# apache/arrow-go

Hardware: AMD Instinct MI355X
Metric: GB/s processed per kernel (Sum/Add/Filter/Take) vs HBM roofline (higher is better)
Workload: dtype int64+f64

## Files before the change

### arrow_go_amd/csrc/ah_common.h

```cpp
#pragma once
#include <hip/hip_runtime.h>
#include <initializer_list>
#include <type_traits>
#include <stdarg.h>
#include <stdint.h>
#include <stddef.h>
#include <stdio.h>
#include <stdlib.h>
#include <string.h>
#include "../../include/arrowhip.h"

#define AH_EXPORT extern "C" __attribute__((visibility("default")))

struct ah_filter_cache {
  bool valid;
  const uint8_t *fdata, *fvalid;
  int64_t foff, n, ntiles;
  int null_sel, tile_rows;
  void* buf;
  size_t bytes;
  int64_t* super_off;
  int* tile_local;
  int64_t* total;
};
// ... 4 lines not shown
  hipStream_t copy_stream;
  bool owns_stream;
  hipEvent_t ev_copy;
  hipEvent_t ev_compute;
  hipEvent_t t0, t1;
  hipEvent_t* marks;
  int n_marks;
  void* scratch;
  size_t scratch_bytes;
  void* temp;
  size_t temp_bytes;
  uint64_t* pinned;
  uint64_t* dscalars;
  int num_cu;
  int tune_nt;
  int tune_blocks_per_cu;
  int opt_take_binned, opt_take_window_log2, opt_take_gather_wg, opt_take_gather_load, opt_take_gather_lds;
  int opt_groupby_keys;
  int opt_groupby_partition;
  int opt_encode_partition;
  int opt_encode_part_slots;
  int opt_encode_byte_map;
  int opt_encode_early_look;
  int opt_encode_part_min;
  int opt_hash_direct;
  int opt_sort_msd;
  int opt_scan_segment_log2;
  void* expr_cache;
  int capturing;
  ah_filter_cache fcache;
  int opt_scan_onepass;
  void* scan_recs;
  size_t scan_recs_bytes;
  unsigned scan_epoch;
  int opt_groupby_seed;
  int opt_groupby_reserve;
  int opt_groupby_lean;
  int opt_filter_cache;
  int take_clustered_hint;
  int opt_take_vec;
  bool take_hint_valid, take_hint_live;
  const void* take_hint_idx; int64_t take_hint_nidx; int take_hint_kind, take_hint_near, take_hint_uses, opt_take_hint_cache;
  unsigned long long take_hint_word;
  int opt_arith_xcd_map;
  int opt_groupby_scale_guess;
  int opt_encode_unperm2_group;
  int opt_encode_resolve_wgs;
  int opt_encode_dict_compact;
  int opt_encode_table_batch;
  int opt_encode_unperm_group;
  int opt_take_vec_nt;
  unsigned long long* mailbox;
  unsigned long long mailbox_seq;
  char err[512];
};

static inline unsigned ah_stream_grid(const ah_ctx* c, int64_t work_items, int default_bpc = 8) {
  int bpc = c->tune_blocks_per_cu > 0 ? c->tune_blocks_per_cu : default_bpc;
  int64_t cap = bpc > 0 ? (int64_t)c->num_cu * bpc : ((int64_t)1 << 30);
  int64_t g = work_items < cap ? work_items : cap;
  return (unsigned)(g < 1 ? 1 : g);
}

static inline int ah_fail(ah_ctx* ctx, int code, const char* fmt, ...) __attribute__((format(printf, 3, 4)));
static inline int ah_fail(ah_ctx* ctx, int code, const char* fmt, ...) {
  if (ctx) {
    va_list ap;
    va_start(ap, fmt);
    vsnprintf(ctx->err, sizeof(ctx->err), fmt, ap);
    va_end(ap);
  }
  return code;
}

#define AH_HIP(ctx, call)                                                              \
  do {                                                                                 \
    hipError_t e__ = (call);                                                           \
    if (e__ != hipSuccess)                                                             \
      return ah_fail((ctx), AH_EHIP, "%s failed: %s (%s:%d)", #call, hipGetErrorString(e__), \
                     __FILE__, __LINE__);                                              \
  } while (0)

#define AH_ENTER_KEEP(ctx)                                             \
  do {                                                                 \
    if (!(ctx)) return AH_EINVALID;                                    \
    (ctx)->err[0] = 0;                                                 \
    AH_HIP((ctx), hipSetDevice((ctx)->device));                        \
  } while (0)

#define AH_ENTER(ctx)                                                  \
  do {                                                                 \
    AH_ENTER_KEEP(ctx);                                                \
    (ctx)->fcache.valid = false;                                       \
    (ctx)->take_hint_valid = false;                                    \
  } while (0)

static inline bool ah_take_hint_overlaps(const ah_ctx* c, const void* p, size_t nbytes) {
  if (!c->take_hint_valid || !c->take_hint_idx) return false;
  const uintptr_t a = (uintptr_t)p, b = a + nbytes, lo = (uintptr_t)c->take_hint_idx, hi = lo + (size_t)c->take_hint_nidx * (size_t)(c->take_hint_kind / 2);
  return a < hi && lo < b;
}
static inline bool ah_fcache_overlaps(const ah_ctx* c, const void* p, size_t nbytes) {
  if (!c->fcache.valid) return false;
  const uintptr_t a = (uintptr_t)p, b = a + nbytes;
  const uintptr_t lo = (uintptr_t)(c->fcache.foff >> 3), hi = (uintptr_t)((c->fcache.foff + c->fcache.n + 7) >> 3);
  for (const uint8_t* bm : {c->fcache.fdata, c->fcache.fvalid})
// ... 131 lines not shown
  for (int j = 0; j < (int)(16 / sizeof(T)); j++) raw[j] = x.v[j];
  __builtin_nontemporal_store(raw, reinterpret_cast<ah_raw16<T>*>(p));
}

template <typename T>
__device__ __forceinline__ ah_vec16<T> ah_ld16(const T* p) {
  const ah_raw16<T> raw = *reinterpret_cast<const ah_raw16<T>*>(p);
  ah_vec16<T> r;
#pragma unroll
  for (int j = 0; j < (int)(16 / sizeof(T)); j++) r.v[j] = raw[j];
  return r;
}
template <typename T>
__device__ __forceinline__ void ah_st16(T* p, const ah_vec16<T>& x) {
  ah_raw16<T> raw;
#pragma unroll
  for (int j = 0; j < (int)(16 / sizeof(T)); j++) raw[j] = x.v[j];
  *reinterpret_cast<ah_raw16<T>*>(p) = raw;
}

template <typename T>
using ah_aligned16 = T __attribute__((ext_vector_type(16 / sizeof(T))));
template <typename ST>
__device__ __forceinline__ ah_vec16<ST> ah_load16(const ST* base, int64_t i, bool aligned) {
  ah_vec16<ST> v;
  if (aligned) {
    const ah_aligned16<ST> t = __builtin_nontemporal_load((const ah_aligned16<ST>*)base + i);
    __builtin_memcpy(&v, &t, 16);
  } else {
    v = ah_ld16<ST>(base + i * (int64_t)(16 / sizeof(ST)));
  }
  return v;
}
template <typename ST>
__device__ __forceinline__ void ah_store16(ST* base, int64_t i, const ah_vec16<ST>& v, bool aligned) {
  if (aligned) {
    ah_aligned16<ST> t;
    __builtin_memcpy(&t, &v, 16);
    __builtin_nontemporal_store(t, (ah_aligned16<ST>*)base + i);
  } else {
    ah_st16<ST>(base + i * (int64_t)(16 / sizeof(ST)), v);
  }
}

template <typename T>
__device__ __forceinline__ T ah_wave_sum(T v) {
#pragma unroll
  for (int o = 32; o > 0; o >>= 1) v += __shfl_down(v, o, 64);
  return v;
}

__device__ __forceinline__ int ah_lane() { return (int)(threadIdx.x & 63); }

__device__ __forceinline__ int ah_bit(const uint8_t* __restrict__ bm, int64_t i) {
  return bm == nullptr ? 1 : (bm[i >> 3] >> (i & 7)) & 1;
}

__device__ __forceinline__ uint64_t ah_load_bits64(const uint8_t* __restrict__ bm, int64_t pos, int nvalid);
__device__ __forceinline__ uint64_t ah_wave_bits64(const uint8_t* __restrict__ bm, int64_t pos0, int64_t nrows_left) {
  const int64_t p = ((int64_t)__builtin_amdgcn_readfirstlane((int)(pos0 >> 32)) << 32) | (unsigned)__builtin_amdgcn_readfirstlane((int)pos0);
  const int64_t left = ((int64_t)__builtin_amdgcn_readfirstlane((int)(nrows_left >> 32)) << 32) | (unsigned)__builtin_amdgcn_readfirstlane((int)nrows_left);
  return ah_load_bits64(bm, p, left >= 64 ? 64 : (int)(left < 0 ? 0 : left));
}
__device__ __forceinline__ uint64_t ah_load_bits64(const uint8_t* __restrict__ bm, int64_t pos, int nvalid) {
  uint64_t mask = nvalid >= 64 ? ~0ull : ((1ull << nvalid) - 1);
  if (nvalid <= 0) return 0;
  if (bm == nullptr) return mask;
  uintptr_t addr = (uintptr_t)bm + (uintptr_t)(pos >> 3);
  uintptr_t base = addr & ~(uintptr_t)7;
  int shift = (int)((addr - base) * 8 + (pos & 7));
  const uint64_t* w = (const uint64_t*)base;
  uint64_t lo = w[0] >> shift;
  if (shift != 0 && shift + nvalid > 64) lo |= w[1] << (64 - shift);
  return lo & mask;
}

__device__ __forceinline__ void put_bits(uint8_t* __restrict__ bm, int64_t pos, unsigned long long word, int cnt) {
  const uintptr_t addr = (uintptr_t)bm + (uintptr_t)(pos >> 3);
  const int sub = (int)(pos & 7);
  if (cnt == 64 && sub == 0 && (addr & 7) == 0) {
    *(unsigned long long*)addr = word;
    return;
  }
  const uintptr_t base = addr & ~(uintptr_t)3;
  int shift = (int)((addr - base) * 8) + sub;
  const unsigned long long m = cnt >= 64 ? ~0ull : ((1ull << cnt) - 1);
  word &= m;
  unsigned* w = (unsigned*)base;
  const unsigned long long mlo = m << shift, vlo = word << shift;
  const unsigned long long mhi = shift ? (m >> (64 - shift)) : 0ull, vhi = shift ? (word >> (64 - shift)) : 0ull;
  const unsigned m0 = (unsigned)mlo, m1 = (unsigned)(mlo >> 32), m2 = (unsigned)mhi;
  const unsigned v0 = (unsigned)vlo, v1 = (unsigned)(vlo >> 32), v2 = (unsigned)vhi;
  if (m0) { atomicAnd(&w[0], ~m0); if (v0) atomicOr(&w[0], v0); }
  if (m1) { atomicAnd(&w[1], ~m1); if (v1) atomicOr(&w[1], v1); }
  if (m2) { atomicAnd(&w[2], ~m2); if (v2) atomicOr(&w[2], v2); }
}

__device__ __forceinline__ void put_word(uint8_t* __restrict__ out, int64_t out_off, int aligned, int64_t chunk, unsigned long long word, int cnt) {
  if (aligned && cnt == 64) *(unsigned long long*)(out + (out_off + chunk * 64) / 8) = word;
  else put_bits(out, out_off + chunk * 64, word, cnt);
}

__device__ __forceinline__ void put_chunk_bytes(uint8_t* __restrict__ bm, int64_t chunk, int64_t n, unsigned long long word) {
  const int64_t left = n - chunk * 64;
  const int nbytes = left >= 64 ? 8 : (int)((left + 7) >> 3);
  for (int b = 0; b < nbytes; b++) bm[chunk * 8 + b] = (uint8_t)(word >> (8 * b));
// ... 2 lines not shown
```

### arrow_go_amd/csrc/ah_ctx.hip

```cpp
#include <chrono>
#include "ah_common.h"

static const char* kVersion = "arrowhip 0.1 (gfx950)";

AH_EXPORT const char* ah_version(void) { return kVersion; }

AH_EXPORT int ah_device_count(int* n_host) {
  int n = 0;
  hipError_t e = hipGetDeviceCount(&n);
  if (n_host) *n_host = (e == hipSuccess) ? n : 0;
  return e == hipSuccess ? AH_OK : AH_EHIP;
}

static int ctx_init_common(ah_ctx* c) {
  AH_HIP(c, hipStreamCreateWithFlags(&c->copy_stream, hipStreamNonBlocking));
  AH_HIP(c, hipEventCreateWithFlags(&c->ev_copy, hipEventDisableTiming));
  AH_HIP(c, hipEventCreateWithFlags(&c->ev_compute, hipEventDisableTiming));
  AH_HIP(c, hipEventCreate(&c->t0));
  AH_HIP(c, hipEventCreate(&c->t1));
  AH_HIP(c, hipHostMalloc((void**)&c->pinned, 64 * sizeof(uint64_t), hipHostMallocDefault));
  AH_HIP(c, hipMalloc((void**)&c->dscalars, (64 + 4096) * sizeof(uint64_t)));
  AH_HIP(c, hipMemset(c->dscalars, 0, (64 + 4096) * sizeof(uint64_t)));
  AH_HIP(c, hipHostMalloc((void**)&c->mailbox, 256, hipHostMallocCoherent | hipHostMallocMapped));
  memset(c->mailbox, 0, 256);
  hipDeviceProp_t prop;
  AH_HIP(c, hipGetDeviceProperties(&prop, c->device));
  c->num_cu = prop.multiProcessorCount > 0 ? prop.multiProcessorCount : 256;
  const char* e_nt = getenv("ARROWHIP_NT");
  c->tune_nt = e_nt ? atoi(e_nt) : 1;
  const char* e_bpc = getenv("ARROWHIP_BLOCKS_PER_CU");
  c->tune_blocks_per_cu = e_bpc ? atoi(e_bpc) : 0;
  auto env_int = [](const char* name, int dflt) { const char* e = getenv(name); return e ? atoi(e) : dflt; };
  c->opt_take_binned = env_int("ARROWHIP_TAKE_BINNED", 1);
  c->opt_take_window_log2 = env_int("ARROWHIP_TAKE_WINDOW_LOG2", 22);
  c->opt_take_gather_wg = env_int("ARROWHIP_TAKE_GATHER_WG_PER_CU", 8);
  c->opt_groupby_partition = env_int("ARROWHIP_GROUPBY_PARTITION", 1);
  c->opt_groupby_keys = env_int("ARROWHIP_GROUPBY_KEYS", 1280);
  c->opt_hash_direct = env_int("ARROWHIP_HASH_DIRECT", 2);
  c->opt_encode_partition = env_int("ARROWHIP_ENCODE_PARTITION", 1);
  c->opt_encode_part_min = env_int("ARROWHIP_ENCODE_PART_MIN", 300000);
  c->opt_encode_early_look = env_int("ARROWHIP_ENCODE_EARLY_LOOK", 1);
  c->opt_encode_byte_map = env_int("ARROWHIP_ENCODE_BYTE_MAP", 1);
  c->opt_encode_part_slots = env_int("ARROWHIP_ENCODE_PART_SLOTS", 8192);
  c->opt_sort_msd = env_int("ARROWHIP_SORT_MSD", 1);
  c->opt_scan_segment_log2 = env_int("ARROWHIP_SCAN_SEGMENT_LOG2", 0);
  c->opt_take_gather_lds = env_int("ARROWHIP_TAKE_GATHER_LDS", 1);
  c->opt_take_vec_nt = env_int("ARROWHIP_TAKE_VEC_NT", 7);
  c->opt_encode_unperm_group = env_int("ARROWHIP_ENCODE_UNPERM_GROUP", 4);
  c->opt_encode_table_batch = env_int("ARROWHIP_ENCODE_TABLE_BATCH", 1);
  c->opt_encode_dict_compact = env_int("ARROWHIP_ENCODE_DICT_COMPACT", 1);
  c->opt_encode_resolve_wgs = env_int("ARROWHIP_ENCODE_RESOLVE_WGS", 1024);
  c->opt_encode_unperm2_group = env_int("ARROWHIP_ENCODE_UNPERM2_GROUP", 4);
  c->opt_groupby_scale_guess = env_int("ARROWHIP_GROUPBY_SCALE_GUESS", 1);
  c->opt_arith_xcd_map = env_int("ARROWHIP_ARITH_XCD_MAP", 0);
  c->opt_take_vec = env_int("ARROWHIP_TAKE_VEC", 1);
  c->opt_take_gather_load = env_int("ARROWHIP_TAKE_GATHER_LOAD", 0);
  return AH_OK;
}

static int ctx_create(int device_id, void* stream, bool borrow, ah_ctx** out) {
  if (!out) return AH_EINVALID;
  *out = nullptr;
  ah_ctx* c = (ah_ctx*)calloc(1, sizeof(ah_ctx));
  if (!c) return AH_EINVALID;
  c->device = device_id;
  hipError_t e = hipSetDevice(device_id);
  if (e != hipSuccess) { free(c); return AH_EHIP; }
  if (borrow) {
    c->stream = (hipStream_t)stream;
    c->owns_stream = false;
  } else {
    e = hipStreamCreateWithFlags(&c->stream, hipStreamNonBlocking);
    if (e != hipSuccess) { free(c); return AH_EHIP; }
    c->owns_stream = true;
  }
  int rc = ctx_init_common(c);
  if (rc != AH_OK) { fprintf(stderr, "arrowhip: ctx init failed: %s\n", c->err); free(c); return rc; }
  c->opt_filter_cache = c->owns_stream ? 1 : 0;
  c->opt_take_hint_cache = c->owns_stream ? 1 : 0;
  c->opt_groupby_lean = 1;
  c->opt_scan_onepass = 1;
  c->opt_groupby_seed = 1;
  c->opt_groupby_reserve = 1;
  *out = c;
  return AH_OK;
}

AH_EXPORT int ah_ctx_create(int device_id, ah_ctx** out) { return ctx_create(device_id, nullptr, false, out); }
AH_EXPORT int ah_ctx_create_on_stream(int device_id, void* hip_stream, ah_ctx** out) {
  return ctx_create(device_id, hip_stream, true, out);
}

AH_EXPORT void ah_ctx_destroy(ah_ctx* c) {
  if (!c) return;
  (void)hipSetDevice(c->device);
  (void)hipStreamSynchronize(c->stream);
  (void)hipStreamSynchronize(c->copy_stream);
  ah_expr_cache_free(c);
  if (c->scratch) (void)hipFree(c->scratch);
  if (c->pinned) (void)hipHostFree(c->pinned);
  if (c->dscalars) (void)hipFree(c->dscalars);
  if (c->mailbox) (void)hipHostFree(c->mailbox);
  if (c->fcache.buf) (void)hipFree(c->fcache.buf);
  if (c->scan_recs) (void)hipFree(c->scan_recs);
  if (c->temp) (void)hipFree(c->temp);
  (void)hipEventDestroy(c->ev_copy);
  (void)hipEventDestroy(c->ev_compute);
  (void)hipEventDestroy(c->t0);
  (void)hipEventDestroy(c->t1);
  for (int i = 0; i < c->n_marks; i++) if (c->marks[i]) (void)hipEventDestroy(c->marks[i]);
  free(c->marks);
  (void)hipStreamDestroy(c->copy_stream);
  if (c->owns_stream) (void)hipStreamDestroy(c->stream);
  free(c);
}

AH_EXPORT int ah_ctx_set_option(ah_ctx* c, const char* name, int64_t value) {
  AH_ENTER(c);
  if (!name) return ah_fail(c, AH_EINVALID, "set_option: null name");
  if (!strcmp(name, "nt")) c->tune_nt = (int)value;
  else if (!strcmp(name, "blocks_per_cu")) c->tune_blocks_per_cu = (int)value;
  else if (!strcmp(name, "take_binned")) c->opt_take_binned = (int)value;
  else if (!strcmp(name, "take_window_log2")) c->opt_take_window_log2 = (int)value;
  else if (!strcmp(name, "take_gather_wg_per_cu")) c->opt_take_gather_wg = (int)value;
  else if (!strcmp(name, "take_gather_lds")) c->opt_take_gather_lds = (int)value;
  else if (!strcmp(name, "take_vec")) c->opt_take_vec = (int)value;
  else if (!strcmp(name, "take_hint_cache")) { c->opt_take_hint_cache = (int)value; c->take_hint_valid = false; }
  else if (!strcmp(name, "take_vec_nt")) c->opt_take_vec_nt = (int)value;
  else if (!strcmp(name, "encode_unperm_group")) c->opt_encode_unperm_group = (int)value;
  else if (!strcmp(name, "encode_table_batch")) c->opt_encode_table_batch = (int)value;
  else if (!strcmp(name, "encode_dict_compact")) c->opt_encode_dict_compact = (int)value;
  else if (!strcmp(name, "encode_unperm2_group")) c->opt_encode_unperm2_group = (int)value;
  else if (!strcmp(name, "encode_resolve_wgs")) c->opt_encode_resolve_wgs = value < 1 ? 1 : (int)value;
  else if (!strcmp(name, "groupby_scale_guess")) c->opt_groupby_scale_guess = (int)value;
  else if (!strcmp(name, "arith_xcd_map")) c->opt_arith_xcd_map = (int)value;
  else if (!strcmp(name, "take_gather_load")) c->opt_take_gather_load = (int)value;
  else if (!strcmp(name, "groupby_partition")) c->opt_groupby_partition = (int)value;
  else if (!strcmp(name, "groupby_keys")) c->opt_groupby_keys = (int)value;
  else if (!strcmp(name, "hash_direct")) c->opt_hash_direct = (int)value;
  else if (!strcmp(name, "encode_partition")) c->opt_encode_partition = (int)value;
  else if (!strcmp(name, "encode_part_min")) c->opt_encode_part_min = (int)value;
  else if (!strcmp(name, "encode_early_look")) c->opt_encode_early_look = (int)value;
  else if (!strcmp(name, "encode_byte_map")) c->opt_encode_byte_map = (int)value;
  else if (!strcmp(name, "encode_part_slots")) c->opt_encode_part_slots = (int)value;
  else if (!strcmp(name, "sort_msd")) c->opt_sort_msd = (int)value;
  else if (!strcmp(name, "scan_onepass")) c->opt_scan_onepass = (int)value;
  else if (!strcmp(name, "groupby_lean")) c->opt_groupby_lean = (int)value;
  else if (!strcmp(name, "groupby_seed")) c->opt_groupby_seed = (int)value;
  else if (!strcmp(name, "groupby_reserve")) c->opt_groupby_reserve = (int)value;
  else if (!strcmp(name, "filter_cache")) { c->opt_filter_cache = value != 0; if (!value) c->fcache.valid = false; }
  else if (!strcmp(name, "scan_segment_log2")) c->opt_scan_segment_log2 = (int)value;
  else return ah_fail(c, AH_EINVALID, "set_option: unknown option '%s'", name);
  return AH_OK;
}

AH_EXPORT const char* ah_last_error(ah_ctx* c) { return c ? c->err : "null context"; }

namespace {
__global__ void mailbox_post_kernel(const unsigned long long* __restrict__ src, int nwords, const unsigned long long* __restrict__ src2, int nwords2,
                                    unsigned long long* mailbox, unsigned long long seq) {
  for (int i = 0; i < nwords; i++) __hip_atomic_store(&mailbox[i], src[i], __ATOMIC_RELAXED, __HIP_MEMORY_SCOPE_SYSTEM);
  for (int i = 0; i < nwords2; i++) __hip_atomic_store(&mailbox[nwords + i], src2[i], __ATOMIC_RELAXED, __HIP_MEMORY_SCOPE_SYSTEM);
  __hip_atomic_store(&mailbox[7], seq, __ATOMIC_RELEASE, __HIP_MEMORY_SCOPE_SYSTEM);
}
}
int ah_mailbox_read(ah_ctx* c, const unsigned long long* dev_words, int nwords, unsigned long long* out_host) {
  return ah_mailbox_read2(c, dev_words, nwords, nullptr, 0, out_host);
}
int ah_mailbox_begin(ah_ctx* c, unsigned long long** mb_out, unsigned long long* seq_out) {
  if (c->capturing) { c->capturing = 2; return ah_fail(c, AH_EINVALID, "this call returns a value to the host: it cannot be recorded into a graph"); }
  *mb_out = c->mailbox + 8;
  *seq_out = ++c->mailbox_seq;
  return AH_OK;
}
int ah_mailbox_wait(ah_ctx* c, unsigned long long seq, int nwords, unsigned long long* out_host) {
  if (nwords < 1 || nwords > 7) return ah_fail(c, AH_EINVALID, "mailbox_wait: 1..7 words");
  unsigned long long* mb = c->mailbox + 8;
  bool seen = false;
  const auto t0 = std::chrono::steady_clock::now();
  for (unsigned spin = 0;; spin++) {
    if (__atomic_load_n(&mb[7], __ATOMIC_ACQUIRE) == seq) { seen = true; break; }
    __builtin_ia32_pause();
    if ((spin & 1023u) == 1023u && std::chrono::steady_clock::now() - t0 > std::chrono::milliseconds(5)) break;
  }
  if (!seen) {
    AH_HIP(c, hipStreamSynchronize(c->stream));
    if (__atomic_load_n(&mb[7], __ATOMIC_ACQUIRE) != seq) return ah_fail(c, AH_EHIP, "mailbox_wait: the kernel did not report");
  }
  for (int i = 0; i < nwords; i++) out_host[i] = __atomic_load_n(&mb[i], __ATOMIC_RELAXED);
  return AH_OK;
}
int ah_mailbox_read2(ah_ctx* c, const unsigned long long* dev_words, int nwords, const unsigned long long* dev_words2, int nwords2,
                     unsigned long long* out_host) {
  if (nwords < 1 || nwords2 < 0 || nwords + nwords2 > 7) return ah_fail(c, AH_EINVALID, "mailbox_read: 1..7 words");
  if (c->capturing) { c->capturing = 2; return ah_fail(c, AH_EINVALID, "this call returns a value to the host: it cannot be recorded into a graph"); }
  unsigned long long* mb = c->mailbox + 8;
  const unsigned long long seq = ++c->mailbox_seq;
  mailbox_post_kernel<<<1, 1, 0, c->stream>>>(dev_words, nwords, dev_words2, nwords2, mb, seq);
// ... 303 lines not shown
```

### arrow_go_amd/csrc/ah_fused.hip

```cpp
#include "ah_common.h"
#include "ah_ddsum.h"

namespace {

constexpr int kBlock = 256;
constexpr int kUnroll = 4;

template <typename T>
using Vec2 = T __attribute__((ext_vector_type(2)));

template <typename T, int OP>
__device__ __forceinline__ bool pred(T a, T t) {
  if (OP == AH_CMP_EQ) return a == t;
  if (OP == AH_CMP_NE) return a != t;
  if (OP == AH_CMP_GT) return a > t;
  return a >= t;
}

struct PartF64 { ah_ddx a; unsigned long long n; };
struct PartI64 { unsigned long long s; unsigned long long n; };

template <typename T> struct Acc;
template <> struct Acc<double> {
  using Part = PartF64;
// ... 30 lines not shown
  }
  __device__ __forceinline__ Part part() const { return Part{s, n}; }
};

template <typename T>
__device__ __forceinline__ void block_reduce(Acc<T>& a, typename Acc<T>::Part* out) {
  __shared__ typename Acc<T>::Part sm[kBlock / 64];
  a.wave_reduce();
  if ((threadIdx.x & 63) == 0) sm[threadIdx.x >> 6] = a.part();
  __syncthreads();
  if (threadIdx.x == 0) {
    Acc<T> r;
#pragma unroll
    for (int w = 0; w < kBlock / 64; w++) r.merge(sm[w]);
    *out = r.part();
  }
}

template <typename T, int OP, bool HAS_VALID, bool NT, bool CAREFUL>
__device__ __forceinline__ unsigned fused_walk(const Vec2<T>* __restrict__ body, int64_t row0, int64_t nvec,
                                               const uint8_t* __restrict__ valid, int64_t off, T thr, Acc<T>& a) {
  unsigned top = 0;
  const int64_t n_iters = (nvec + (int64_t)kBlock * kUnroll - 1) / ((int64_t)kBlock * kUnroll);
  for (int64_t it = blockIdx.x; it < n_iters; it += gridDim.x) {
    const int64_t base = it * kBlock * kUnroll + threadIdx.x;
    const bool full = (it + 1) * (int64_t)kBlock * kUnroll <= nvec;
    Vec2<T> v[kUnroll];
    if (full) {
#pragma unroll
      for (int k = 0; k < kUnroll; k++) {
        if (NT) v[k] = __builtin_nontemporal_load(&body[base + (int64_t)k * kBlock]);
        else v[k] = body[base + (int64_t)k * kBlock];
      }
    }
#pragma unroll
    for (int k = 0; k < kUnroll; k++) {
      const int64_t j = base + (int64_t)k * kBlock;
      if (!full) {
        if (j >= nvec) continue;
        v[k] = body[j];
      }
      unsigned vb = 3;
      if (HAS_VALID) {
        const int64_t bit = off + row0 + 2 * j;
        vb = (unsigned)((valid[bit >> 3] >> (bit & 7)) & 1) | ((unsigned)((valid[(bit + 1) >> 3] >> ((bit + 1) & 7)) & 1) << 1);
      }
      if ((vb & 1) && pred<T, OP>(v[k].x, thr)) { if (CAREFUL) a.add(v[k].x); else top = max(top, a.add_small(v[k].x)); }
      if ((vb & 2) && pred<T, OP>(v[k].y, thr)) { if (CAREFUL) a.add(v[k].y); else top = max(top, a.add_small(v[k].y)); }
    }
  }
  return top;
}

template <typename T, int OP, bool HAS_VALID, bool NT>
__global__ __launch_bounds__(kBlock) void fused_kernel(const T* __restrict__ x, int64_t n, int64_t row0, int64_t nvec,
                                                        const uint8_t* __restrict__ valid, int64_t off, T thr,
                                                        typename Acc<T>::Part* __restrict__ partials) {
  Acc<T> a;
  const Vec2<T>* body = (const Vec2<T>*)(x + row0);
  const unsigned top = fused_walk<T, OP, HAS_VALID, NT, !Acc<T>::kClassed>(body, row0, nvec, valid, off, thr, a);
  if (Acc<T>::kClassed && __any(top >= AH_DDX_BIG_HI)) {
    a = Acc<T>();
    (void)fused_walk<T, OP, HAS_VALID, NT, true>(body, row0, nvec, valid, off, thr, a);
  }
  if (blockIdx.x == 0 && threadIdx.x == 0) {
    for (int64_t i = 0; i < row0; i++)
      if ((!HAS_VALID || ah_bit(valid, off + i)) && pred<T, OP>(x[i], thr)) a.add(x[i]);
    for (int64_t i = row0 + 2 * nvec; i < n; i++)
      if ((!HAS_VALID || ah_bit(valid, off + i)) && pred<T, OP>(x[i], thr)) a.add(x[i]);
  }
  block_reduce<T>(a, &partials[blockIdx.x]);
}

template <typename T>
__global__ __launch_bounds__(kBlock) void fused_final_kernel(const typename Acc<T>::Part* __restrict__ partials, int np,
                                                              T* __restrict__ out_sum, int64_t* __restrict__ out_count,
                                                              double* __restrict__ out_parts) {
  Acc<T> a;
  for (int i = threadIdx.x; i < np; i += kBlock) a.merge(partials[i]);
  __shared__ typename Acc<T>::Part res;
  block_reduce<T>(a, &res);
  __syncthreads();
  if (threadIdx.x == 0) {
    if constexpr (__is_floating_point(T)) {
      *out_sum = ah_ddx_result(res.a);
      if (out_parts) { out_parts[0] = res.a.s; out_parts[1] = res.a.e; out_parts[2] = res.a.bs; out_parts[3] = res.a.be; }
    } else {
      *out_sum = (T)res.s;
    }
    *out_count = (int64_t)res.n;
  }
}

template <typename T>
int fused_dev(ah_ctx* c, int cmpop, const T* x, const uint8_t* valid, int64_t off, int64_t n, T thr, T* out_sum_dev,
              int64_t* out_count_dev, double* out_parts_dev = nullptr) {
  if (n < 0 || off < 0) return ah_fail(c, AH_EINVALID, "cmp_filter_sum: negative length/offset");
  if (n == 0) {
    AH_HIP(c, hipMemsetAsync(out_sum_dev, 0, sizeof(T), c->stream));
    AH_HIP(c, hipMemsetAsync(out_count_dev, 0, sizeof(int64_t), c->stream));
    if (out_parts_dev) AH_HIP(c, hipMemsetAsync(out_parts_dev, 0, 4 * sizeof(double), c->stream));
    return AH_OK;
  }
  if (!x) return ah_fail(c, AH_EINVALID, "cmp_filter_sum: null values");
  if ((uintptr_t)x & 7) return ah_fail(c, AH_EINVALID, "cmp_filter_sum: buffer not element-aligned");
  int64_t row0 = ((uintptr_t)x & 15) ? 1 : 0;
  if (row0 > n) row0 = n;
  int64_t nvec = (n - row0) / 2;
  unsigned grid = ah_stream_grid(c, ah_ceil_div(nvec > 0 ? nvec : 1, (int64_t)kBlock * kUnroll), valid ? 8 : 2);
  using Part = typename Acc<T>::Part;
  void* scratch;
  int rc = ah_scratch_reserve(c, (size_t)grid * sizeof(Part), &scratch);
  if (rc != AH_OK) return rc;
  Part* partials = (Part*)scratch;
#define AH_FUSED(OPC)                                                                                                   \
  if (valid) {                                                                                                          \
    if (c->tune_nt) fused_kernel<T, OPC, true, true><<<grid, kBlock, 0, c->stream>>>(x, n, row0, nvec, valid, off, thr, partials);   \
    else fused_kernel<T, OPC, true, false><<<grid, kBlock, 0, c->stream>>>(x, n, row0, nvec, valid, off, thr, partials);             \
  } else {                                                                                                              \
    if (c->tune_nt) fused_kernel<T, OPC, false, true><<<grid, kBlock, 0, c->stream>>>(x, n, row0, nvec, valid, off, thr, partials);  \
    else fused_kernel<T, OPC, false, false><<<grid, kBlock, 0, c->stream>>>(x, n, row0, nvec, valid, off, thr, partials);            \
  }
  switch (cmpop) {
    case AH_CMP_EQ: AH_FUSED(AH_CMP_EQ) break;
    case AH_CMP_NE: AH_FUSED(AH_CMP_NE) break;
    case AH_CMP_GT: AH_FUSED(AH_CMP_GT) break;
    case AH_CMP_GE: AH_FUSED(AH_CMP_GE) break;
    default: return ah_fail(c, AH_EINVALID, "cmp_filter_sum: bad op %d", cmpop);
  }
#undef AH_FUSED
  AH_LAUNCH_CHECK(c);
  fused_final_kernel<T><<<1, kBlock, 0, c->stream>>>(partials, (int)grid, out_sum_dev, out_count_dev, out_parts_dev);
  AH_LAUNCH_CHECK(c);
  return AH_OK;
}

template <typename T>
int fused_host(ah_ctx* c, int cmpop, const T* x, const uint8_t* valid, int64_t off, int64_t n, T thr, T* out_sum_host,
               int64_t* out_count_host) {
  T* dsum = (T*)&c->dscalars[8];
  int64_t* dcnt = (int64_t*)&c->dscalars[9];
  int rc = fused_dev<T>(c, cmpop, x, valid, off, n, thr, dsum, dcnt);
  if (rc != AH_OK) return rc;
  { int mrc = ah_mailbox_read(c, (const unsigned long long*)dsum, 2, (unsigned long long*)c->pinned); if (mrc != AH_OK) return mrc; }
  if (out_sum_host) memcpy(out_sum_host, (const void*)&c->pinned[0], sizeof(T));
  if (out_count_host) memcpy(out_count_host, (const void*)&c->pinned[1], sizeof(int64_t));
  return AH_OK;
}

}

AH_EXPORT int ah_cmp_filter_sum_i64(ah_ctx* c, int cmpop, const int64_t* x, const uint8_t* valid, int64_t off, int64_t n,
                                    int64_t threshold, int64_t* out_sum_host, int64_t* out_count_host) {
  AH_ENTER(c);
  return fused_host<int64_t>(c, cmpop, x, valid, off, n, threshold, out_sum_host, out_count_host);
}
AH_EXPORT int ah_cmp_filter_sum_f64(ah_ctx* c, int cmpop, const double* x, const uint8_t* valid, int64_t off, int64_t n,
                                    double threshold, double* out_sum_host, int64_t* out_count_host) {
  AH_ENTER(c);
  return fused_host<double>(c, cmpop, x, valid, off, n, threshold, out_sum_host, out_count_host);
}
AH_EXPORT int ah_cmp_filter_sum_i64_dev(ah_ctx* c, int cmpop, const int64_t* x, const uint8_t* valid, int64_t off,
                                        int64_t n, int64_t threshold, int64_t* out_sum_count_dev) {
  AH_ENTER(c);
  if (!out_sum_count_dev) return ah_fail(c, AH_EINVALID, "cmp_filter_sum: null output");
  return fused_dev<int64_t>(c, cmpop, x, valid, off, n, threshold, out_sum_count_dev, out_sum_count_dev + 1);
}
AH_EXPORT int ah_cmp_filter_sum_f64_dev(ah_ctx* c, int cmpop, const double* x, const uint8_t* valid, int64_t off,
                                        int64_t n, double threshold, double* out_sum_dev, int64_t* out_count_dev) {
  AH_ENTER(c);
  if (!out_sum_dev || !out_count_dev) return ah_fail(c, AH_EINVALID, "cmp_filter_sum: null output");
  return fused_dev<double>(c, cmpop, x, valid, off, n, threshold, out_sum_dev, out_count_dev);
}
int ah_fused_f64_parts_dev(ah_ctx* c, int cmpop, const double* x, const uint8_t* valid, int64_t off, int64_t n, double threshold,
                           double* out_sum_dev, int64_t* out_count_dev, double* out_parts_dev) {
  return fused_dev<double>(c, cmpop, x, valid, off, n, threshold, out_sum_dev, out_count_dev, out_parts_dev);
}
```

### arrow_go_amd/csrc/ah_minmax.hip

```cpp
#include <limits>
#include "ah_common.h"

namespace {

constexpr int kBlock = 256;
constexpr int kUnroll = 4;

template <typename T>
struct MM {
  T lo, hi;
  __device__ __forceinline__ void init() { lo = std::numeric_limits<T>::max(); hi = std::numeric_limits<T>::min(); }
  __device__ __forceinline__ void add(T v) { lo = v < lo ? v : lo; hi = v > hi ? v : hi; }
  __device__ __forceinline__ void merge(const MM& o) { lo = o.lo < lo ? o.lo : lo; hi = o.hi > hi ? o.hi : hi; }
};

template <typename T>
__device__ __forceinline__ MM<T> block_reduce(MM<T> a) {
  using W = typename std::conditional<sizeof(T) == 8, long long, int>::type;
#pragma unroll
  for (int o = 32; o > 0; o >>= 1) {
    MM<T> b;
    b.lo = (T)__shfl_down((W)a.lo, o, 64);
    b.hi = (T)__shfl_down((W)a.hi, o, 64);
    a.merge(b);
  }
  __shared__ MM<T> sm[kBlock / 64];
  if ((threadIdx.x & 63) == 0) sm[threadIdx.x >> 6] = a;
  __syncthreads();
  if (threadIdx.x == 0)
    for (int w = 1; w < kBlock / 64; w++) a.merge(sm[w]);
  return a;
}

template <typename T, bool NT>
__global__ __launch_bounds__(kBlock) void minmax_partials_kernel(const T* __restrict__ values, int64_t n, MM<T>* __restrict__ partials) {
  constexpr int V = 16 / sizeof(T);
  typedef unsigned u32x4 __attribute__((ext_vector_type(4)));
  MM<T> a;
  a.init();
  const uintptr_t addr = (uintptr_t)values;
  int64_t head = ((16 - (addr & 15)) & 15) / sizeof(T);
  if (head > n) head = n;
  const int64_t nvec = (n - head) / V;
  const u32x4* body = (const u32x4*)(values + head);
  const int64_t stride = (int64_t)gridDim.x * kBlock * kUnroll;
  for (int64_t i = (int64_t)blockIdx.x * kBlock * kUnroll + threadIdx.x; i < nvec; i += stride) {
    u32x4 v[kUnroll];
#pragma unroll
    for (int k = 0; k < kUnroll; k++) {
      const int64_t j = i + (int64_t)k * kBlock;
      if (j < nvec) v[k] = NT ? __builtin_nontemporal_load(&body[j]) : body[j];
    }
#pragma unroll
    for (int k = 0; k < kUnroll; k++) {
      if (i + (int64_t)k * kBlock < nvec) {
        const ah_vec16<T> e = __builtin_bit_cast(ah_vec16<T>, v[k]);
#pragma unroll
        for (int j = 0; j < V; j++) a.add(e.v[j]);
      }
    }
  }
  if (blockIdx.x == 0 && threadIdx.x == 0) {
    for (int64_t k = 0; k < head; k++) a.add(values[k]);
    for (int64_t k = head + nvec * V; k < n; k++) a.add(values[k]);
  }
  a = block_reduce<T>(a);
  if (threadIdx.x == 0) partials[blockIdx.x] = a;
}

template <typename T>
__global__ __launch_bounds__(kBlock) void minmax_final_kernel(const MM<T>* __restrict__ partials, int np, T* __restrict__ out ) {
  MM<T> a;
  a.init();
  for (int i = threadIdx.x; i < np; i += kBlock) a.merge(partials[i]);
  a = block_reduce<T>(a);
  if (threadIdx.x == 0) { out[0] = a.lo; out[1] = a.hi; }
}

template <typename T>
int run_minmax(ah_ctx* c, const void* values, int64_t n, void* out_min_host, void* out_max_host) {
  const unsigned grid = ah_stream_grid(c, ah_ceil_div(ah_ceil_div(n, 16 / sizeof(T)), (int64_t)kBlock * kUnroll), 2);
  void* scratch;
  int rc = ah_scratch_reserve(c, (size_t)grid * sizeof(MM<T>) + 64, &scratch);
  if (rc != AH_OK) return rc;
  MM<T>* partials = (MM<T>*)scratch;
  T* res = (T*)&c->dscalars[12];
  if (c->tune_nt) minmax_partials_kernel<T, true><<<grid, kBlock, 0, c->stream>>>((const T*)values, n, partials);
  else minmax_partials_kernel<T, false><<<grid, kBlock, 0, c->stream>>>((const T*)values, n, partials);
  AH_LAUNCH_CHECK(c);
  minmax_final_kernel<T><<<1, kBlock, 0, c->stream>>>(partials, (int)grid, res);
  AH_LAUNCH_CHECK(c);
  AH_HIP(c, hipMemcpyAsync(c->pinned, res, 2 * sizeof(T), hipMemcpyDeviceToHost, c->stream));
  AH_HIP(c, hipStreamSynchronize(c->stream));
  memcpy(out_min_host, (const void*)c->pinned, sizeof(T));
  memcpy(out_max_host, (const uint8_t*)c->pinned + sizeof(T), sizeof(T));
  return AH_OK;
}

}

AH_EXPORT int ah_min_max(ah_ctx* c, int type, const void* values, int64_t n, void* out_min_host, void* out_max_host) {
  AH_ENTER(c);
  if (n < 0) return ah_fail(c, AH_EINVALID, "min_max: negative length");
  if (!out_min_host || !out_max_host) return ah_fail(c, AH_EINVALID, "min_max: null result pointer");
  const int w = ah_type_width(type);
  if (!w || type == AH_FLOAT32 || type == AH_FLOAT64) return ah_fail(c, AH_ENOTIMPL, "min_max: integer types only (got %d)", type);
  if (n > 0 && (!values || ((uintptr_t)values & (uintptr_t)(w - 1)))) return ah_fail(c, AH_EINVALID, "min_max: null or misaligned buffer");
  switch (type) {
#define AH_MM(ID, T)                                                                                              \
  case ID: {                                                                                                      \
    if (n == 0) { T lo = std::numeric_limits<T>::max(), hi = std::numeric_limits<T>::min();                     \
                  memcpy(out_min_host, &lo, sizeof(T)); memcpy(out_max_host, &hi, sizeof(T)); return AH_OK; }     \
    return run_minmax<T>(c, values, n, out_min_host, out_max_host);                                               \
  }
    AH_MM(AH_UINT8, uint8_t) AH_MM(AH_INT8, int8_t) AH_MM(AH_UINT16, uint16_t) AH_MM(AH_INT16, int16_t)
    AH_MM(AH_UINT32, uint32_t) AH_MM(AH_INT32, int32_t) AH_MM(AH_UINT64, uint64_t) AH_MM(AH_INT64, int64_t)
#undef AH_MM
  }
  return ah_fail(c, AH_ENOTIMPL, "min_max: integer types only (got %d)", type);
}
```

### arrow_go_amd/csrc/ah_sum.hip

```cpp
#include "ah_common.h"
#include "ah_ddsum.h"

namespace {

constexpr int kBlock = 256;
constexpr int kUnroll = 4;

struct AccDD {
  ah_ddx a;
  __device__ __forceinline__ void init() { ah_ddx_init(a); }
  __device__ __forceinline__ void add(double x) { ah_ddx_add(a, x); }
  __device__ __forceinline__ void add_small(double x) { ah_dd_add(a.s, a.e, x); }
  __device__ __forceinline__ void merge(const AccDD& o) { ah_ddx_merge(a, o.a); }
  __device__ __forceinline__ void wave_reduce() {
#pragma unroll
    for (int o = 32; o > 0; o >>= 1) {
      ah_ddx t;
      t.s = __shfl_down(a.s, o, 64);
      t.e = __shfl_down(a.e, o, 64);
      t.bs = __shfl_down(a.bs, o, 64);
      t.be = __shfl_down(a.be, o, 64);
      ah_ddx_merge(a, t);
    }
  }
// ... 23 lines not shown
using Vec2 = T __attribute__((ext_vector_type(2)));

template <typename Acc>
__device__ __forceinline__ void block_reduce_store(Acc acc, Acc* out) {
  __shared__ Acc sm[kBlock / 64];
  acc.wave_reduce();
  int lane = threadIdx.x & 63, wave = threadIdx.x >> 6;
  if (lane == 0) sm[wave] = acc;
  __syncthreads();
  if (threadIdx.x == 0) {
    Acc a = sm[0];
#pragma unroll
    for (int w = 1; w < kBlock / 64; w++) a.merge(sm[w]);
    *out = a;
  }
}

template <typename T, typename Acc, bool NT, bool CAREFUL>
__device__ __forceinline__ unsigned sum_walk(const Vec2<T>* __restrict__ body, int64_t nvec, Acc& a0, Acc& a1) {
  unsigned top = 0;
  const int64_t stride = (int64_t)gridDim.x * kBlock * kUnroll;
  int64_t i = (int64_t)blockIdx.x * kBlock * kUnroll + threadIdx.x;
  for (; i + (int64_t)(kUnroll - 1) * kBlock < nvec; i += stride) {
    Vec2<T> v[kUnroll];
#pragma unroll
    for (int k = 0; k < kUnroll; k++) {
      if (NT) v[k] = __builtin_nontemporal_load(&body[i + (int64_t)k * kBlock]);
      else v[k] = body[i + (int64_t)k * kBlock];
    }
#pragma unroll
    for (int k = 0; k < kUnroll; k++) {
      if (CAREFUL) {
        a0.add(v[k].x);
        a1.add(v[k].y);
      } else {
        a0.add_small(v[k].x);
        a1.add_small(v[k].y);
        top = max(top, max(Acc::hi_abs(v[k].x), Acc::hi_abs(v[k].y)));
      }
    }
  }
#pragma unroll
  for (int k = 0; k < kUnroll; k++) {
    int64_t j = i + (int64_t)k * kBlock;
    if (j < nvec) {
      Vec2<T> v = body[j];
      a0.add(v.x);
      a1.add(v.y);
    }
  }
  return top;
}

template <typename T, typename Acc, bool NT>
__global__ __launch_bounds__(kBlock) void sum_partials_kernel(const Vec2<T>* __restrict__ body, int64_t nvec,
                                                               const T* __restrict__ head, int nhead,
                                                               const T* __restrict__ tail, int ntail,
                                                               Acc* __restrict__ partials) {
  Acc a0, a1;
  a0.init();
  a1.init();
  const unsigned top = sum_walk<T, Acc, NT, false>(body, nvec, a0, a1);
  if (Acc::kClassed && __any(top >= Acc::kBigHi)) {
    a0.init();
    a1.init();
    (void)sum_walk<T, Acc, NT, true>(body, nvec, a0, a1);
  }
  if (blockIdx.x == 0 && threadIdx.x == 0) {
    for (int k = 0; k < nhead; k++) a0.add(head[k]);
    for (int k = 0; k < ntail; k++) a1.add(tail[k]);
  }
  a0.merge(a1);
  block_reduce_store(a0, &partials[blockIdx.x]);
}

template <typename T, typename Acc>
__global__ __launch_bounds__(kBlock) void sum_final_kernel(const Acc* __restrict__ partials, int n, T* __restrict__ out) {
  Acc a;
  a.init();
  for (int i = threadIdx.x; i < n; i += kBlock) a.merge(partials[i]);
  __shared__ Acc res;
  block_reduce_store(a, &res);
  __syncthreads();
  if (threadIdx.x == 0) *out = (T)res.result();
}

constexpr size_t kSeqRows = 31;
__global__ void sum_seq_f64_kernel(const double* __restrict__ buf, int n, double* __restrict__ out) {
  double acc = 0.0;
  for (int i = 0; i < n; i++) acc += buf[i];
  *out = acc;
}

template <typename T, typename Acc>
int sum_dev(ah_ctx* c, const T* buf, size_t len, T* res_dev) {
  if (len == 0) {
    AH_HIP(c, hipMemsetAsync(res_dev, 0, sizeof(T), c->stream));
    return AH_OK;
  }
  if (((uintptr_t)buf & (sizeof(T) - 1)) != 0) return ah_fail(c, AH_EINVALID, "sum: buffer not element-aligned");
  if constexpr (Acc::kClassed) {
    if (len <= kSeqRows) {
      sum_seq_f64_kernel<<<1, 1, 0, c->stream>>>((const double*)buf, (int)len, (double*)res_dev);
      AH_LAUNCH_CHECK(c);
      return AH_OK;
    }
  }
  int nhead = (int)((((uintptr_t)buf & 15) != 0) ? 1 : 0);
  if ((size_t)nhead > len) nhead = (int)len;
  const T* body = buf + nhead;
  int64_t nvec = (int64_t)((len - nhead) / 2);
  const T* tail = body + nvec * 2;
  int ntail = (int)(len - nhead - (size_t)nvec * 2);
  int64_t iters = ah_ceil_div(nvec, (int64_t)kBlock * kUnroll);
  unsigned grid = ah_stream_grid(c, iters, 2);
  void* scratch;
  int rc = ah_scratch_reserve(c, (size_t)grid * sizeof(Acc), &scratch);
  if (rc != AH_OK) return rc;
  Acc* partials = (Acc*)scratch;
  if (c->tune_nt)
    sum_partials_kernel<T, Acc, true><<<grid, kBlock, 0, c->stream>>>((const Vec2<T>*)body, nvec, buf, nhead, tail, ntail, partials);
  else
    sum_partials_kernel<T, Acc, false><<<grid, kBlock, 0, c->stream>>>((const Vec2<T>*)body, nvec, buf, nhead, tail, ntail, partials);
  AH_LAUNCH_CHECK(c);
  sum_final_kernel<T, Acc><<<1, kBlock, 0, c->stream>>>(partials, (int)grid, res_dev);
  AH_LAUNCH_CHECK(c);
  return AH_OK;
}

template <typename T, typename Acc>
int sum_chunk(ah_ctx* c, const T* buf, size_t len, Acc* partials, int max_partials, int* n_written) {
  *n_written = 0;
  if (len == 0) return AH_OK;
  if (((uintptr_t)buf & (sizeof(T) - 1)) != 0) return ah_fail(c, AH_EINVALID, "sum: buffer not element-aligned");
  int nhead = (int)((((uintptr_t)buf & 15) != 0) ? 1 : 0);
  if ((size_t)nhead > len) nhead = (int)len;
  const T* body = buf + nhead;
  const int64_t nvec = (int64_t)((len - nhead) / 2);
  const T* tail = body + nvec * 2;
  const int ntail = (int)(len - nhead - (size_t)nvec * 2);
  unsigned grid = ah_stream_grid(c, ah_ceil_div(nvec, (int64_t)kBlock * kUnroll), 2);
  if ((int)grid > max_partials) grid = (unsigned)max_partials;
  if (c->tune_nt)
    sum_partials_kernel<T, Acc, true><<<grid, kBlock, 0, c->stream>>>((const Vec2<T>*)body, nvec, buf, nhead, tail, ntail, partials);
  else
    sum_partials_kernel<T, Acc, false><<<grid, kBlock, 0, c->stream>>>((const Vec2<T>*)body, nvec, buf, nhead, tail, ntail, partials);
  AH_LAUNCH_CHECK(c);
  *n_written = (int)grid;
  return AH_OK;
}

template <typename T, typename Acc>
int sum_host(ah_ctx* c, const T* buf, size_t len, T* res_host) {
  if (!res_host) return ah_fail(c, AH_EINVALID, "sum: null result pointer");
  if (len == 0) { *res_host = 0; return AH_OK; }
  T* dres = (T*)c->dscalars;
  int rc = sum_dev<T, Acc>(c, buf, len, dres);
  if (rc != AH_OK) return rc;
  static_assert(sizeof(T) == 8, "one mailbox word");
  if ((rc = ah_mailbox_read(c, (const unsigned long long*)dres, 1, (unsigned long long*)c->pinned)) != AH_OK) return rc;
  memcpy(res_host, c->pinned, sizeof(T));
  return AH_OK;
}

}

size_t ah_sum_partial_bytes(int is_f64) { return is_f64 ? sizeof(AccDD) : sizeof(AccU64); }
int ah_sum_chunk_partials(ah_ctx* c, int is_f64, const void* buf, size_t len, void* partials, int max_partials, int* n_written) {
  if (is_f64) return sum_chunk<double, AccDD>(c, (const double*)buf, len, (AccDD*)partials, max_partials, n_written);
  return sum_chunk<uint64_t, AccU64>(c, (const uint64_t*)buf, len, (AccU64*)partials, max_partials, n_written);
}
int ah_sum_short_f64(ah_ctx* c, const void* buf, size_t len, void* res_dev) {
  return sum_dev<double, AccDD>(c, (const double*)buf, len, (double*)res_dev);
}
int ah_sum_finish_partials(ah_ctx* c, int is_f64, const void* partials, int n, void* res_dev) {
  if (n <= 0) { AH_HIP(c, hipMemsetAsync(res_dev, 0, 8, c->stream)); return AH_OK; }
  if (is_f64) sum_final_kernel<double, AccDD><<<1, kBlock, 0, c->stream>>>((const AccDD*)partials, n, (double*)res_dev);
  else sum_final_kernel<uint64_t, AccU64><<<1, kBlock, 0, c->stream>>>((const AccU64*)partials, n, (uint64_t*)res_dev);
  AH_LAUNCH_CHECK(c);
  return AH_OK;
}

AH_EXPORT int ah_sum_float64(ah_ctx* c, const double* buf, size_t len, double* res_host) {
  AH_ENTER(c);
  return sum_host<double, AccDD>(c, buf, len, res_host);
}
AH_EXPORT int ah_sum_int64(ah_ctx* c, const int64_t* buf, size_t len, int64_t* res_host) {
  AH_ENTER(c);
  return sum_host<uint64_t, AccU64>(c, (const uint64_t*)buf, len, (uint64_t*)res_host);
}
AH_EXPORT int ah_sum_uint64(ah_ctx* c, const uint64_t* buf, size_t len, uint64_t* res_host) {
  AH_ENTER(c);
  return sum_host<uint64_t, AccU64>(c, buf, len, res_host);
}
AH_EXPORT int ah_sum_float64_dev(ah_ctx* c, const double* buf, size_t len, double* res_dev) {
  AH_ENTER(c);
  return sum_dev<double, AccDD>(c, buf, len, res_dev);
}
AH_EXPORT int ah_sum_int64_dev(ah_ctx* c, const int64_t* buf, size_t len, int64_t* res_dev) {
// ... 4 lines not shown
```

Before: 6239.

## Fuse final reduction into partials kernel via last-workgroup atomic ticket

Sum, minmax and fused filter-sum reductions now finish inside the partials kernel. Each workgroup takes an atomic ticket after writing its partial, and the last one merges all partials and writes the result. This removes the second single-block launch and its launch gap. The cost is a device-scope fence and atomic per workgroup, plus a shared ticket counter that must wrap back to zero correctly across calls.

```diff
diff --git a/arrow_go_amd/csrc/ah_common.h b/arrow_go_amd/csrc/ah_common.h
--- a/arrow_go_amd/csrc/ah_common.h
+++ b/arrow_go_amd/csrc/ah_common.h
@@ -80,6 +80,8 @@
   int opt_take_vec_nt;
   unsigned long long* mailbox;
   unsigned long long mailbox_seq;
+  unsigned* reduce_ticket;
+  int opt_reduce_one_launch;
   char err[512];
 };
 
@@ -317,6 +319,25 @@
 
 __device__ __forceinline__ int ah_lane() { return (int)(threadIdx.x & 63); }
 
+__device__ __forceinline__ bool ah_last_workgroup(unsigned* __restrict__ ticket) {
+  if (gridDim.x == 1) {
+    __syncthreads();
+    return true;
+  }
+  __shared__ unsigned last;
+  if (threadIdx.x == 0) {
+    __builtin_amdgcn_fence(__ATOMIC_RELEASE, "agent");
+    const bool l = atomicInc(ticket, gridDim.x - 1) == gridDim.x - 1;
+    if (l) {
+      __builtin_amdgcn_fence(__ATOMIC_ACQUIRE, "agent");
+      __builtin_amdgcn_s_waitcnt(0x0F70);
+    }
+    last = l;
+  }
+  __syncthreads();
+  return last != 0;
+}
+
 __device__ __forceinline__ int ah_bit(const uint8_t* __restrict__ bm, int64_t i) {
   return bm == nullptr ? 1 : (bm[i >> 3] >> (i & 7)) & 1;
 }
diff --git a/arrow_go_amd/csrc/ah_ctx.hip b/arrow_go_amd/csrc/ah_ctx.hip
--- a/arrow_go_amd/csrc/ah_ctx.hip
+++ b/arrow_go_amd/csrc/ah_ctx.hip
@@ -23,6 +23,8 @@
   AH_HIP(c, hipMemset(c->dscalars, 0, (64 + 4096) * sizeof(uint64_t)));
   AH_HIP(c, hipHostMalloc((void**)&c->mailbox, 256, hipHostMallocCoherent | hipHostMallocMapped));
   memset(c->mailbox, 0, 256);
+  AH_HIP(c, hipMalloc((void**)&c->reduce_ticket, 256));
+  AH_HIP(c, hipMemset(c->reduce_ticket, 0, 256));
   hipDeviceProp_t prop;
   AH_HIP(c, hipGetDeviceProperties(&prop, c->device));
   c->num_cu = prop.multiProcessorCount > 0 ? prop.multiProcessorCount : 256;
@@ -54,6 +56,7 @@
   c->opt_groupby_scale_guess = env_int("ARROWHIP_GROUPBY_SCALE_GUESS", 1);
   c->opt_arith_xcd_map = env_int("ARROWHIP_ARITH_XCD_MAP", 0);
   c->opt_take_vec = env_int("ARROWHIP_TAKE_VEC", 1);
+  c->opt_reduce_one_launch = env_int("ARROWHIP_REDUCE_ONE_LAUNCH", 1);
   c->opt_take_gather_load = env_int("ARROWHIP_TAKE_GATHER_LOAD", 0);
   return AH_OK;
 }
@@ -103,6 +106,7 @@
   if (c->mailbox) (void)hipHostFree(c->mailbox);
   if (c->fcache.buf) (void)hipFree(c->fcache.buf);
   if (c->scan_recs) (void)hipFree(c->scan_recs);
+  if (c->reduce_ticket) (void)hipFree(c->reduce_ticket);
   if (c->temp) (void)hipFree(c->temp);
   (void)hipEventDestroy(c->ev_copy);
   (void)hipEventDestroy(c->ev_compute);
@@ -144,6 +148,7 @@
   else if (!strcmp(name, "encode_byte_map")) c->opt_encode_byte_map = (int)value;
   else if (!strcmp(name, "encode_part_slots")) c->opt_encode_part_slots = (int)value;
   else if (!strcmp(name, "sort_msd")) c->opt_sort_msd = (int)value;
+  else if (!strcmp(name, "reduce_one_launch")) c->opt_reduce_one_launch = value != 0;
   else if (!strcmp(name, "scan_onepass")) c->opt_scan_onepass = (int)value;
   else if (!strcmp(name, "groupby_lean")) c->opt_groupby_lean = (int)value;
   else if (!strcmp(name, "groupby_seed")) c->opt_groupby_seed = (int)value;
diff --git a/arrow_go_amd/csrc/ah_fused.hip b/arrow_go_amd/csrc/ah_fused.hip
--- a/arrow_go_amd/csrc/ah_fused.hip
+++ b/arrow_go_amd/csrc/ah_fused.hip
@@ -106,30 +106,9 @@
   return top;
 }
 
-template <typename T, int OP, bool HAS_VALID, bool NT>
-__global__ __launch_bounds__(kBlock) void fused_kernel(const T* __restrict__ x, int64_t n, int64_t row0, int64_t nvec,
-                                                        const uint8_t* __restrict__ valid, int64_t off, T thr,
-                                                        typename Acc<T>::Part* __restrict__ partials) {
-  Acc<T> a;
-  const Vec2<T>* body = (const Vec2<T>*)(x + row0);
-  const unsigned top = fused_walk<T, OP, HAS_VALID, NT, !Acc<T>::kClassed>(body, row0, nvec, valid, off, thr, a);
-  if (Acc<T>::kClassed && __any(top >= AH_DDX_BIG_HI)) {
-    a = Acc<T>();
-    (void)fused_walk<T, OP, HAS_VALID, NT, true>(body, row0, nvec, valid, off, thr, a);
-  }
-  if (blockIdx.x == 0 && threadIdx.x == 0) {
-    for (int64_t i = 0; i < row0; i++)
-      if ((!HAS_VALID || ah_bit(valid, off + i)) && pred<T, OP>(x[i], thr)) a.add(x[i]);
-    for (int64_t i = row0 + 2 * nvec; i < n; i++)
-      if ((!HAS_VALID || ah_bit(valid, off + i)) && pred<T, OP>(x[i], thr)) a.add(x[i]);
-  }
-  block_reduce<T>(a, &partials[blockIdx.x]);
-}
-
-template <typename T>
-__global__ __launch_bounds__(kBlock) void fused_final_kernel(const typename Acc<T>::Part* __restrict__ partials, int np,
-                                                              T* __restrict__ out_sum, int64_t* __restrict__ out_count,
-                                                              double* __restrict__ out_parts) {
+template <typename T>
+__device__ __forceinline__ void fused_finish(const typename Acc<T>::Part* partials, int np, T* __restrict__ out_sum,
+                                             int64_t* __restrict__ out_count, double* __restrict__ out_parts) {
   Acc<T> a;
   for (int i = threadIdx.x; i < np; i += kBlock) a.merge(partials[i]);
   __shared__ typename Acc<T>::Part res;
@@ -147,6 +126,42 @@
 }
 
 template <typename T>
+struct FusedOut {
+  unsigned* ticket;
+  T* sum;
+  int64_t* count;
+  double* parts;
+};
+
+template <typename T, int OP, bool HAS_VALID, bool NT>
+__global__ __launch_bounds__(kBlock) void fused_kernel(const T* __restrict__ x, int64_t n, int64_t row0, int64_t nvec,
+                                                        const uint8_t* __restrict__ valid, int64_t off, T thr,
+                                                        typename Acc<T>::Part* partials, FusedOut<T> o) {
+  Acc<T> a;
+  const Vec2<T>* body = (const Vec2<T>*)(x + row0);
+  const unsigned top = fused_walk<T, OP, HAS_VALID, NT, !Acc<T>::kClassed>(body, row0, nvec, valid, off, thr, a);
+  if (Acc<T>::kClassed && __any(top >= AH_DDX_BIG_HI)) {
+    a = Acc<T>();
+    (void)fused_walk<T, OP, HAS_VALID, NT, true>(body, row0, nvec, valid, off, thr, a);
+  }
+  if (blockIdx.x == 0 && threadIdx.x == 0) {
+    for (int64_t i = 0; i < row0; i++)
+      if ((!HAS_VALID || ah_bit(valid, off + i)) && pred<T, OP>(x[i], thr)) a.add(x[i]);
+    for (int64_t i = row0 + 2 * nvec; i < n; i++)
+      if ((!HAS_VALID || ah_bit(valid, off + i)) && pred<T, OP>(x[i], thr)) a.add(x[i]);
+  }
+  block_reduce<T>(a, &partials[blockIdx.x]);
+  if (o.ticket != nullptr && ah_last_workgroup(o.ticket)) fused_finish<T>(partials, (int)gridDim.x, o.sum, o.count, o.parts);
+}
+
+template <typename T>
+__global__ __launch_bounds__(kBlock) void fused_final_kernel(const typename Acc<T>::Part* __restrict__ partials, int np,
+                                                              T* __restrict__ out_sum, int64_t* __restrict__ out_count,
+                                                              double* __restrict__ out_parts) {
+  fused_finish<T>(partials, np, out_sum, out_count, out_parts);
+}
+
+template <typename T>
 int fused_dev(ah_ctx* c, int cmpop, const T* x, const uint8_t* valid, int64_t off, int64_t n, T thr, T* out_sum_dev,
               int64_t* out_count_dev, double* out_parts_dev = nullptr) {
   if (n < 0 || off < 0) return ah_fail(c, AH_EINVALID, "cmp_filter_sum: negative length/offset");
@@ -167,13 +182,14 @@
   int rc = ah_scratch_reserve(c, (size_t)grid * sizeof(Part), &scratch);
   if (rc != AH_OK) return rc;
   Part* partials = (Part*)scratch;
+  const FusedOut<T> o = {c->opt_reduce_one_launch ? c->reduce_ticket : nullptr, out_sum_dev, out_count_dev, out_parts_dev};
 #define AH_FUSED(OPC)                                                                                                   \
   if (valid) {                                                                                                          \
-    if (c->tune_nt) fused_kernel<T, OPC, true, true><<<grid, kBlock, 0, c->stream>>>(x, n, row0, nvec, valid, off, thr, partials);   \
-    else fused_kernel<T, OPC, true, false><<<grid, kBlock, 0, c->stream>>>(x, n, row0, nvec, valid, off, thr, partials);             \
+    if (c->tune_nt) fused_kernel<T, OPC, true, true><<<grid, kBlock, 0, c->stream>>>(x, n, row0, nvec, valid, off, thr, partials, o);   \
+    else fused_kernel<T, OPC, true, false><<<grid, kBlock, 0, c->stream>>>(x, n, row0, nvec, valid, off, thr, partials, o);             \
   } else {                                                                                                              \
-    if (c->tune_nt) fused_kernel<T, OPC, false, true><<<grid, kBlock, 0, c->stream>>>(x, n, row0, nvec, valid, off, thr, partials);  \
-    else fused_kernel<T, OPC, false, false><<<grid, kBlock, 0, c->stream>>>(x, n, row0, nvec, valid, off, thr, partials);            \
+    if (c->tune_nt) fused_kernel<T, OPC, false, true><<<grid, kBlock, 0, c->stream>>>(x, n, row0, nvec, valid, off, thr, partials, o);  \
+    else fused_kernel<T, OPC, false, false><<<grid, kBlock, 0, c->stream>>>(x, n, row0, nvec, valid, off, thr, partials, o);            \
   }
   switch (cmpop) {
     case AH_CMP_EQ: AH_FUSED(AH_CMP_EQ) break;
@@ -184,6 +200,7 @@
   }
 #undef AH_FUSED
   AH_LAUNCH_CHECK(c);
+  if (o.ticket) return AH_OK;
   fused_final_kernel<T><<<1, kBlock, 0, c->stream>>>(partials, (int)grid, out_sum_dev, out_count_dev, out_parts_dev);
   AH_LAUNCH_CHECK(c);
   return AH_OK;
diff --git a/arrow_go_amd/csrc/ah_minmax.hip b/arrow_go_amd/csrc/ah_minmax.hip
--- a/arrow_go_amd/csrc/ah_minmax.hip
+++ b/arrow_go_amd/csrc/ah_minmax.hip
@@ -32,8 +32,18 @@
   return a;
 }
 
+template <typename T>
+__device__ __forceinline__ void minmax_finish(const MM<T>* partials, int np, T* __restrict__ out ) {
+  MM<T> a;
+  a.init();
+  for (int i = threadIdx.x; i < np; i += kBlock) a.merge(partials[i]);
+  a = block_reduce<T>(a);
+  if (threadIdx.x == 0) { out[0] = a.lo; out[1] = a.hi; }
+}
+
 template <typename T, bool NT>
-__global__ __launch_bounds__(kBlock) void minmax_partials_kernel(const T* __restrict__ values, int64_t n, MM<T>* __restrict__ partials) {
+__global__ __launch_bounds__(kBlock) void minmax_partials_kernel(const T* __restrict__ values, int64_t n, MM<T>* partials,
+                                                                  unsigned* __restrict__ ticket, T* __restrict__ out) {
   constexpr int V = 16 / sizeof(T);
   typedef unsigned u32x4 __attribute__((ext_vector_type(4)));
   MM<T> a;
@@ -66,15 +76,12 @@
   }
   a = block_reduce<T>(a);
   if (threadIdx.x == 0) partials[blockIdx.x] = a;
+  if (ticket != nullptr && ah_last_workgroup(ticket)) minmax_finish<T>(partials, (int)gridDim.x, out);
 }
 
 template <typename T>
 __global__ __launch_bounds__(kBlock) void minmax_final_kernel(const MM<T>* __restrict__ partials, int np, T* __restrict__ out ) {
-  MM<T> a;
-  a.init();
-  for (int i = threadIdx.x; i < np; i += kBlock) a.merge(partials[i]);
-  a = block_reduce<T>(a);
-  if (threadIdx.x == 0) { out[0] = a.lo; out[1] = a.hi; }
+  minmax_finish<T>(partials, np, out);
 }
 
 template <typename T>
@@ -85,11 +92,14 @@
   if (rc != AH_OK) return rc;
   MM<T>* partials = (MM<T>*)scratch;
   T* res = (T*)&c->dscalars[12];
-  if (c->tune_nt) minmax_partials_kernel<T, true><<<grid, kBlock, 0, c->stream>>>((const T*)values, n, partials);
-  else minmax_partials_kernel<T, false><<<grid, kBlock, 0, c->stream>>>((const T*)values, n, partials);
+  unsigned* ticket = c->opt_reduce_one_launch ? c->reduce_ticket : nullptr;
+  if (c->tune_nt) minmax_partials_kernel<T, true><<<grid, kBlock, 0, c->stream>>>((const T*)values, n, partials, ticket, res);
+  else minmax_partials_kernel<T, false><<<grid, kBlock, 0, c->stream>>>((const T*)values, n, partials, ticket, res);
   AH_LAUNCH_CHECK(c);
-  minmax_final_kernel<T><<<1, kBlock, 0, c->stream>>>(partials, (int)grid, res);
-  AH_LAUNCH_CHECK(c);
+  if (!ticket) {
+    minmax_final_kernel<T><<<1, kBlock, 0, c->stream>>>(partials, (int)grid, res);
+    AH_LAUNCH_CHECK(c);
+  }
   AH_HIP(c, hipMemcpyAsync(c->pinned, res, 2 * sizeof(T), hipMemcpyDeviceToHost, c->stream));
   AH_HIP(c, hipStreamSynchronize(c->stream));
   memcpy(out_min_host, (const void*)c->pinned, sizeof(T));
diff --git a/arrow_go_amd/csrc/ah_sum.hip b/arrow_go_amd/csrc/ah_sum.hip
--- a/arrow_go_amd/csrc/ah_sum.hip
+++ b/arrow_go_amd/csrc/ah_sum.hip
@@ -99,11 +99,23 @@
   return top;
 }
 
+template <typename T, typename Acc>
+__device__ __forceinline__ void sum_finish(const Acc* partials, int n, T* __restrict__ out) {
+  Acc a;
+  a.init();
+  for (int i = threadIdx.x; i < n; i += kBlock) a.merge(partials[i]);
+  __shared__ Acc res;
+  block_reduce_store(a, &res);
+  __syncthreads();
+  if (threadIdx.x == 0) *out = (T)res.result();
+}
+
 template <typename T, typename Acc, bool NT>
 __global__ __launch_bounds__(kBlock) void sum_partials_kernel(const Vec2<T>* __restrict__ body, int64_t nvec,
                                                                const T* __restrict__ head, int nhead,
                                                                const T* __restrict__ tail, int ntail,
-                                                               Acc* __restrict__ partials) {
+                                                               Acc* partials, unsigned* __restrict__ ticket,
+                                                               T* __restrict__ out) {
   Acc a0, a1;
   a0.init();
   a1.init();
@@ -119,17 +131,12 @@
   }
   a0.merge(a1);
   block_reduce_store(a0, &partials[blockIdx.x]);
+  if (ticket != nullptr && ah_last_workgroup(ticket)) sum_finish<T, Acc>(partials, (int)gridDim.x, out);
 }
 
 template <typename T, typename Acc>
 __global__ __launch_bounds__(kBlock) void sum_final_kernel(const Acc* __restrict__ partials, int n, T* __restrict__ out) {
-  Acc a;
-  a.init();
-  for (int i = threadIdx.x; i < n; i += kBlock) a.merge(partials[i]);
-  __shared__ Acc res;
-  block_reduce_store(a, &res);
-  __syncthreads();
-  if (threadIdx.x == 0) *out = (T)res.result();
+  sum_finish<T, Acc>(partials, n, out);
 }
 
 constexpr size_t kSeqRows = 31;
@@ -165,11 +172,13 @@
   int rc = ah_scratch_reserve(c, (size_t)grid * sizeof(Acc), &scratch);
   if (rc != AH_OK) return rc;
   Acc* partials = (Acc*)scratch;
+  unsigned* ticket = c->opt_reduce_one_launch ? c->reduce_ticket : nullptr;
   if (c->tune_nt)
-    sum_partials_kernel<T, Acc, true><<<grid, kBlock, 0, c->stream>>>((const Vec2<T>*)body, nvec, buf, nhead, tail, ntail, partials);
+    sum_partials_kernel<T, Acc, true><<<grid, kBlock, 0, c->stream>>>((const Vec2<T>*)body, nvec, buf, nhead, tail, ntail, partials, ticket, res_dev);
   else
-    sum_partials_kernel<T, Acc, false><<<grid, kBlock, 0, c->stream>>>((const Vec2<T>*)body, nvec, buf, nhead, tail, ntail, partials);
-  AH_LAUNCH_CHECK(c);
+    sum_partials_kernel<T, Acc, false><<<grid, kBlock, 0, c->stream>>>((const Vec2<T>*)body, nvec, buf, nhead, tail, ntail, partials, ticket, res_dev);
+  AH_LAUNCH_CHECK(c);
+  if (ticket) return AH_OK;
   sum_final_kernel<T, Acc><<<1, kBlock, 0, c->stream>>>(partials, (int)grid, res_dev);
   AH_LAUNCH_CHECK(c);
   return AH_OK;
@@ -189,9 +198,9 @@
   unsigned grid = ah_stream_grid(c, ah_ceil_div(nvec, (int64_t)kBlock * kUnroll), 2);
   if ((int)grid > max_partials) grid = (unsigned)max_partials;
   if (c->tune_nt)
-    sum_partials_kernel<T, Acc, true><<<grid, kBlock, 0, c->stream>>>((const Vec2<T>*)body, nvec, buf, nhead, tail, ntail, partials);
+    sum_partials_kernel<T, Acc, true><<<grid, kBlock, 0, c->stream>>>((const Vec2<T>*)body, nvec, buf, nhead, tail, ntail, partials, nullptr, nullptr);
   else
-    sum_partials_kernel<T, Acc, false><<<grid, kBlock, 0, c->stream>>>((const Vec2<T>*)body, nvec, buf, nhead, tail, ntail, partials);
+    sum_partials_kernel<T, Acc, false><<<grid, kBlock, 0, c->stream>>>((const Vec2<T>*)body, nvec, buf, nhead, tail, ntail, partials, nullptr, nullptr);
   AH_LAUNCH_CHECK(c);
   *n_written = (int)grid;
   return AH_OK;
```

Result: slower. 6064 (-2.8%).
